# rlog58/dags-vae-search

Hardware: AMD Instinct MI355X
Metric: DAGs/sec VAE+predictor train step, n=12 batch 4096 per GPU, at 1 MI355X (higher is better)
Workload: dtype f32 (fwd bf16x6, bwd bf16x3 split products, fp32 accumulate); 1 GPU; synthetic_v12 DAGs (n=12, card=12, N=15 tokens), PACE-VAE train step: pack + fwd + bwd + clip_grad_norm_(1.0) + Adam(1e-4), train mode dropout 0.15; per_gpu_batch=4096, global_batch=4096, waves_per_workgroup=8, parallelism=single

## Files before the change

dags_vae_search_amd/csrc/dvs_api.hip:

```cpp
#include <math.h>
#include <stdarg.h>
#include <stdio.h>
#include <stdlib.h>
#include <string.h>

#include "dvs_kernels.h"
#include "dvs_backward.h"
#include "dvs_wide.h"
#include "dvs_wimg.h"
#include "dvs_decode.h"
#include "dvs_search_args.h"

static thread_local char g_err[256] = "";

#include <map>
#include <mutex>
#include <string>
#include <utility>
#include <vector>
namespace {
struct ProfRec {
    const char* name;
#ifndef DVS_EMU
    hipEvent_t a, b;
// ... 446 lines not shown
    return call_end("dvs_build_records");
}

static inline int slot_enc(int layer, int sub) { return 1 + 2 * layer + sub; }
static inline int slot_dec(int layer, int sub) { return 8 + 3 * layer + sub; }
static inline int site_enc(int layer, int k) { return 4 + 4 * layer + k; }
static inline int site_dec(int layer, int k) { return 16 + 6 * layer + k; }

static inline size_t img_attn(int block) { return (size_t)block * DvsAttnImg::SIZE; }
static inline size_t img_ffn(int block) { return DVS_N_ATTN_BLOCKS * DvsAttnImg::SIZE + (size_t)block * DvsFfnImg::SIZE; }
static inline int blk_enc_attn(int layer) { return layer; }
static inline int blk_dec_self(int layer) { return 3 + 2 * layer; }
static inline int blk_dec_cross(int layer) { return 4 + 2 * layer; }
static inline int blk_enc_ffn(int layer) { return layer; }
static inline int blk_dec_ffn(int layer) { return 3 + layer; }

static inline const void* wimg_attn(const Step& c, int block) { return (const dvs_bf16*)(c.ws + c.W.wimg) + img_attn(block); }
static inline const void* wimg_ffn(const Step& c, int block) { return (const dvs_bf16*)(c.ws + c.W.wimg) + img_ffn(block); }

static DvsLN ln_of(const Step& c, int slot, const DvsNormP* n) {
    if (!n) return DvsLN{nullptr, nullptr, nullptr};
    return DvsLN{c.ws + c.W.stats[slot], c.P + n->w, c.P + n->b};
}

static EmbedArgs embed_args(const Step& c, int site) {
    EmbedArgs e;
    memset(&e, 0, sizeof(e));
    e.dims = c.d;
    e.rec = c.rec;
    e.W1 = c.P + c.L.W1;
    e.W2 = c.P + c.L.W2;
    e.lab_w = c.P + c.L.lab_w;
    e.lab_b = c.P + c.L.lab_b;
    e.embimg = (const float*)((const dvs_bf16*)(c.ws + c.W.wimg) + DVS_WIMG_EMB);
    e.site = site;
    return e;
}

static AttnArgs attn_args(const Step& c, const DvsAttnP& p, int block, int in, const DvsNormP* norm, const float* kv, int out,
                          int site0) {
    AttnArgs a;
    memset(&a, 0, sizeof(a));
    a.dims = c.d;
    a.rec = c.rec;
    a.xin = c.ws + c.W.act[in];
    a.ln = ln_of(c, in, norm);
    a.kv = kv;
    a.in_w = c.P + p.in_w;
    a.in_b = c.P + p.in_b;
    a.out_w = c.P + p.out_w;
    a.out_b = c.P + p.out_b;
    a.wimg = wimg_attn(c, block);
    a.qkv = c.wide ? c.ws + c.W.qkv[block] : nullptr;
    a.out_pre = c.ws + c.W.act[out];
    a.out_stats = c.ws + c.W.stats[out];
    a.site_prob = site0;
    a.site_post = site0 + 1;
    return a;
}

static FfnArgs ffn_args(const Step& c, const DvsFfnP& p, int block, int in, const DvsNormP& norm, int out, int site0) {
    FfnArgs f;
    memset(&f, 0, sizeof(f));
    f.dims = c.d;
    f.xin = c.ws + c.W.act[in];
    f.ln = ln_of(c, in, &norm);
    f.l1_w = c.P + p.l1_w;
// ... 92 lines not shown
        attn(L.enc[i].sa, blk_enc_attn(i));
        ffn(L.enc[i].ff, blk_enc_ffn(i));
        attn(L.dec[i].sa, blk_dec_self(i));
        attn(L.dec[i].ca, blk_dec_cross(i));
        ffn(L.dec[i].ff, blk_dec_ffn(i));
    }
    if (!wide) {
        add(L.edge0_w, DVS_WIMG_LOSS + DvsLossImg::Wa, 64, 8);
        add(L.edge0_w + 64, DVS_WIMG_LOSS + DvsLossImg::Wb, 64, 8);
        add(L.edge0_w, DVS_WIMG_LOSS + DvsLossImg::WaT, 64, 8 | 1);
        add(L.edge0_w + 64, DVS_WIMG_LOSS + DvsLossImg::WbT, 64, 8 | 1);
    }
    dvs_bf16* wimg = (dvs_bf16*)(c.ws + c.W.wimg);
    DvsLatImgArgs lat;
    lat.fc1_w = c.P + L.fc1_w;
    lat.fc2_w = c.P + L.fc2_w;
    lat.fc3_w = c.P + L.fc3_w;
    lat.fc3_b = c.P + L.fc3_b;
    lat.img = c.ws + c.W.limg;
    lat.N = c.d.N;
    lat.NT = c.d.NT;
    DvsLossHeadArgs head;
    memset(&head, 0, sizeof(head));
    if (!wide) {
        head_params(c, head);
        head.ln_g = c.P + L.dec[DVS_LAYERS - 1].n3.w;
        head.ln_b = c.P + L.dec[DVS_LAYERS - 1].n3.b;
        head.dst = (float*)(wimg + DVS_WIMG_LOSS + DvsLossImg::Head);
        head.C = c.d.C;
        head.W1 = c.P + L.W1;
        head.W2 = c.P + L.W2;
        head.lab_w = c.P + L.lab_w;
        head.lab_b = c.P + L.lab_b;
        head.dst_emb = (float*)(wimg + DVS_WIMG_EMB);
        head.N = c.d.N;
    }
    dvs_launch_prepare_images(J, c.P, wimg, lat, head, c.st);
}

static void launch_embed_fwd(const Step& c, const EmbedArgs& e) {
    if (c.wide) dvs_launch_embed_fwd_w(e, c.g.tiles4, c.st);
    else if (c.nw == 4) dvs_launch_embed_fwd(e, c.g.chain, 4, c.st);
    else dvs_launch_embed_fwd(e, c.g.tiles16, 16, c.st);
}
static void launch_attn_fwd(const Step& c, const AttnArgs& a) {
    if (c.wide) dvs_launch_attn_fwd_w(a, c.g.dags, c.st);
    else if (c.nw == 4) dvs_launch_attn_fwd(a, c.g.chain, 4, c.st);
    else dvs_launch_attn_fwd(a, c.g.tiles8, 8, c.st);
}
static void launch_ffn_fwd(const Step& c, const FfnArgs& f) {
    if (c.nw == 4) dvs_launch_ffn_fwd(f, c.g.chain, 4, c.st);
    else dvs_launch_ffn_fwd(f, c.g.tiles16, 16, c.st);
}
static void launch_loss_fwd(const Step& c, const LossArgs& a) {
    if (c.wide) dvs_launch_loss_fwd_w(a, c.g.dags2, c.st);
    else if (c.nw == 4) dvs_launch_loss_fwd(a, c.g.chain, 4, c.st);
    else dvs_launch_loss_fwd(a, c.g.tiles8, 8, c.st);
}
struct FwdChain {
    FwdStackArgs stack;
    const Step& c;
    int tag;
    bool chain;
    FwdChain(const Step& step, int tag_) : c(step), tag(tag_), chain(!step.wide && !split_stack()) { memset(&stack, 0, sizeof(stack)); }
    FwdPhase& next(int kind) {
        if (stack.nphase == DVS_FWD_STACK_PHASES) flush();
        FwdPhase& ph = stack.ph[stack.nphase++];
// ... 221 lines not shown
```

dags_vae_search_amd/csrc/dvs_bf16.h:

```cpp
#pragma once
#include "dvs_device.h"

typedef __bf16 dvs_bf16;
typedef __bf16 bf8 __attribute__((ext_vector_type(8)));

constexpr int DVS_LDB = 72;

__device__ __forceinline__ f4 dvs_mfma_bf(bf8 a, bf8 b, f4 c) { return __builtin_amdgcn_mfma_f32_16x16x32_bf16(a, b, c, 0, 0, 0); }

__device__ __forceinline__ int dvs_kperm(int f) {
    const int t = f >> 4, g = (f >> 2) & 3, kk = f & 3;
    return 32 * (t >> 1) + 8 * g + 4 * (t & 1) + kk;
}

__device__ __forceinline__ void dvs_split1(float v, dvs_bf16& hi, dvs_bf16& lo) {
    hi = (dvs_bf16)v;
    lo = (dvs_bf16)(v - (float)hi);
}
__device__ __forceinline__ void dvs_split8(const f4& a, const f4& b, bf8& hi, bf8& lo) {
#pragma unroll
    for (int i = 0; i < 4; ++i) {
        dvs_bf16 h, l;
        dvs_split1(a[i], h, l);
        hi[i] = h;
        lo[i] = l;
        dvs_split1(b[i], h, l);
        hi[4 + i] = h;
        lo[4 + i] = l;
    }
}
struct SplitT {
    bf8 hi[2], lo[2];
};
__device__ __forceinline__ SplitT dvs_split_T(const f4 (&x)[4]) {
    SplitT s;
    dvs_split8(x[0], x[1], s.hi[0], s.lo[0]);
    dvs_split8(x[2], x[3], s.hi[1], s.lo[1]);
    return s;
}

__device__ __forceinline__ bf8 dvs_wfrag(const dvs_bf16* img, int row, int p, const Lane& L) {
    return *(const bf8*)(img + row * DVS_LDB + 32 * p + 8 * L.g);
}

template <int OT>
__device__ __forceinline__ void dvs_matb_T(f4 (&y)[OT], const SplitT& x, const dvs_bf16* Wh, const dvs_bf16* Wl, int row0,
                                           const Lane& L) {
#pragma unroll
    for (int p = 0; p < 2; ++p) {
        bf8 ah[OT], al[OT];
#pragma unroll
        for (int ot = 0; ot < OT; ++ot) {
            ah[ot] = dvs_wfrag(Wh, row0 + 16 * ot + L.r, p, L);
            al[ot] = dvs_wfrag(Wl, row0 + 16 * ot + L.r, p, L);
        }
#pragma unroll
        for (int ot = 0; ot < OT; ++ot) y[ot] = dvs_mfma_bf(ah[ot], x.hi[p], y[ot]);
#pragma unroll
        for (int ot = 0; ot < OT; ++ot) y[ot] = dvs_mfma_bf(ah[ot], x.lo[p], y[ot]);
#pragma unroll
        for (int ot = 0; ot < OT; ++ot) y[ot] = dvs_mfma_bf(al[ot], x.hi[p], y[ot]);
        DVS_SCHED_FENCE();
    }
}
template <int OT>
__device__ __forceinline__ void dvs_matb_N(f4 (&y)[OT], const SplitT& x, const dvs_bf16* Wh, const dvs_bf16* Wl, int row0,
                                           const Lane& L) {
#pragma unroll
    for (int p = 0; p < 2; ++p) {
        bf8 bh[OT], bl[OT];
#pragma unroll
        for (int ot = 0; ot < OT; ++ot) {
            bh[ot] = dvs_wfrag(Wh, row0 + 16 * ot + L.r, p, L);
            bl[ot] = dvs_wfrag(Wl, row0 + 16 * ot + L.r, p, L);
        }
#pragma unroll
        for (int ot = 0; ot < OT; ++ot) y[ot] = dvs_mfma_bf(x.hi[p], bh[ot], y[ot]);
#pragma unroll
        for (int ot = 0; ot < OT; ++ot) y[ot] = dvs_mfma_bf(x.lo[p], bh[ot], y[ot]);
#pragma unroll
        for (int ot = 0; ot < OT; ++ot) y[ot] = dvs_mfma_bf(x.hi[p], bl[ot], y[ot]);
        DVS_SCHED_FENCE();
    }
}

struct Split3T {
    bf8 hi[2], mid[2], lo[2];
// ... 18 lines not shown
            dvs_split3_1(x[2 * p + 1][i], h, m, l);
            s.hi[p][4 + i] = h;
            s.mid[p][4 + i] = m;
            s.lo[p][4 + i] = l;
        }
    return s;
}
template <int OT, bool N_LAYOUT = false>
__device__ __forceinline__ void dvs_matb3(f4 (&y)[OT], const Split3T& x, const dvs_bf16* img, int rows, int row0, const Lane& L) {
    const dvs_bf16* Wh = img;
    const dvs_bf16* Wm = img + rows * DVS_LDB;
    const dvs_bf16* Wl = Wm + rows * DVS_LDB;
#pragma unroll
    for (int p = 0; p < 2; ++p) {
        bf8 wh[OT], wm[OT], wl[OT];
#pragma unroll
        for (int ot = 0; ot < OT; ++ot) {
            wh[ot] = dvs_wfrag(Wh, row0 + 16 * ot + L.r, p, L);
            wm[ot] = dvs_wfrag(Wm, row0 + 16 * ot + L.r, p, L);
            wl[ot] = dvs_wfrag(Wl, row0 + 16 * ot + L.r, p, L);
        }
#define DVS_M3(wa, xa)                                                                                     \
    _Pragma("unroll") for (int ot = 0; ot < OT; ++ot)                                                      \
        y[ot] = N_LAYOUT ? dvs_mfma_bf(xa[p], wa[ot], y[ot]) : dvs_mfma_bf(wa[ot], xa[p], y[ot]);
        DVS_M3(wl, x.hi)
        DVS_M3(wh, x.lo)
        DVS_M3(wm, x.mid)
        DVS_M3(wm, x.hi)
        DVS_M3(wh, x.mid)
        DVS_M3(wh, x.hi)
#undef DVS_M3
        DVS_SCHED_FENCE();
    }
}

typedef __bf16 bf4 __attribute__((ext_vector_type(4)));
constexpr int DVS_PLD = 68;
constexpr int DVS_PKB = 16 * DVS_PLD;

__device__ __forceinline__ void dvs_park_bf(dvs_bf16* img, const f4 (&x)[4], const Lane& L) {
#pragma unroll
    for (int t = 0; t < 4; ++t) {
        bf4 h, l;
#pragma unroll
        for (int i = 0; i < 4; ++i) {
            dvs_bf16 hh, ll;
            dvs_split1(x[t][i], hh, ll);
            h[i] = hh;
            l[i] = ll;
        }
        *(bf4*)(img + L.r * DVS_PLD + 16 * t + 4 * L.g) = h;
        *(bf4*)(img + DVS_PKB + L.r * DVS_PLD + 16 * t + 4 * L.g) = l;
    }
}
__device__ __forceinline__ bf4 dvs_tr_read(const dvs_bf16* p) {
#ifndef DVS_EMU
    typedef short s4_ __attribute__((ext_vector_type(4)));
    const s4_ v = __builtin_amdgcn_ds_read_tr16_b64_v4i16((s4_ __attribute__((address_space(3)))*)p);
    return __builtin_bit_cast(bf4, v);
#else
    const unsigned long long a = (unsigned long long)p;
    const int lane = (int)(threadIdx.x & 63), grp = lane & 48, i = lane & 15;
    bf4 out;
    for (int q = 0; q < 4; ++q) {
        const int src = grp + 4 * q + (i >> 2);
        const unsigned lo = __shfl((unsigned)(a & 0xFFFFFFFFull), src), hi = __shfl((unsigned)(a >> 32), src);
// ... 47 lines not shown
```

dags_vae_search_amd/csrc/dvs_kernels.h:

```cpp
#pragma once
#include "dvs_device.h"
#include "dvs_host.h"
#include "dvs_stage.h"

#ifndef DVS_EMU
typedef hipStream_t dvs_stream_t;
#else
typedef void* dvs_stream_t;
#endif

struct DvsLN {
    const float* stats;
    const float* g;
    const float* b;
};

struct PackArgs {
    int B, N, C;
    const float* lab1h;
    const float* pos1h;
    const float* adj;
    const uint8_t* tmask;
    DvsRecord* rec;
    int* status;
};

struct EmbedArgs {
    DvsDims dims;
    const DvsRecord* rec;
    const float *W1, *W2, *lab_w, *lab_b;
    const float* embimg;
    float* out;
    int site;
    float* out2;
    int site2;
    const float* gout;
    float* slab;
    int64_t P;
    int64_t oW1, oW2, olab_w, olab_b;
};

struct AttnArgs {
    DvsDims dims;
    const DvsRecord* rec;
    const float* xin;
    DvsLN ln;
    const float* kv;
    const float *in_w, *in_b, *out_w, *out_b;
    const void* wimg;
    float* out_pre;
    float* out_stats;
    int site_prob, site_post;
    float* qkv;
};

struct FfnArgs {
    DvsDims dims;
    const float* xin;
    DvsLN ln;
    const float *l1_w, *l1_b, *l2_w, *l2_b;
    const void* wimg;
    float* out_pre;
    float* out_stats;
    float* out_norm;
// ... 236 lines not shown
```

dags_vae_search_amd/csrc/dvs_wimg.h:

```cpp
#pragma once
#include "dvs_bf16.h"

constexpr size_t DVS_IMG64 = 64 * (size_t)DVS_LDB;
struct DvsAttnImg {
    static constexpr size_t Win = 0;
    static constexpr size_t Wout = 3 * 3 * DVS_IMG64;
    static constexpr size_t WoutT = Wout + 3 * DVS_IMG64;
    static constexpr size_t WinB = WoutT + 2 * DVS_IMG64;
    static constexpr size_t WinT = WinB + 2 * 3 * DVS_IMG64;
    static constexpr size_t SIZE = WinT + 3 * 2 * DVS_IMG64;
};
struct DvsFfnImg {
    static constexpr size_t W2T = 0;
    static constexpr size_t W1T = 2 * DVS_IMG64;
    static constexpr size_t W1 = 4 * DVS_IMG64;
    static constexpr size_t W2 = 7 * DVS_IMG64;
    static constexpr size_t SIZE = 10 * DVS_IMG64;
};
struct DvsLossImg {
    static constexpr size_t Wa = 0;
    static constexpr size_t Wb = 3 * DVS_IMG64;
    static constexpr size_t WaT = 6 * DVS_IMG64;
    static constexpr size_t WbT = 8 * DVS_IMG64;
    static constexpr size_t Head = 10 * DVS_IMG64;
    static constexpr int HEAD_FLOATS = 32 * 68 + 16 * 36 + 32 + 16 + 64 + 64 + 16 + 64 + 64;
    static constexpr size_t SIZE = Head + 2 * (size_t)HEAD_FLOATS;
};
static_assert(DvsLossImg::HEAD_FLOATS % 256 == 0 && DVS_LD == 68, "whole 1 KB chunks (dvs_stage.h)");
struct DvsEmbImg {
    static constexpr int FLOATS = 5120;
};
struct DvsLossHeadArgs {
    const float *node0_w, *node0_b, *node2_w, *node2_b, *edge0_b, *edge2_w, *edge2_b, *ln_g, *ln_b;
    float* dst;
    int C;
    const float *W1, *W2, *lab_w, *lab_b;
    float* dst_emb;
    int N;
};
constexpr int DVS_N_ATTN_BLOCKS = 9, DVS_N_FFN_BLOCKS = 6;
constexpr size_t DVS_WIMG_LOSS = DVS_N_ATTN_BLOCKS * DvsAttnImg::SIZE + DVS_N_FFN_BLOCKS * DvsFfnImg::SIZE;
constexpr size_t DVS_WIMG_EMB = DVS_WIMG_LOSS + DvsLossImg::SIZE;
constexpr size_t DVS_WIMG_BF16 = DVS_WIMG_EMB + 2 * (size_t)DvsEmbImg::FLOATS;

struct DvsLatImg {
    static constexpr size_t LD(int NT) { return (size_t)1024 * NT + 64; }
    static constexpr size_t A(int) { return 0; }
    static constexpr size_t AT(int NT) { return 64 * LD(NT); }
    static constexpr size_t W3(int NT) { return AT(NT) + (size_t)64 * 1024 * NT; }
    static constexpr size_t W3T(int NT) { return W3(NT) + (size_t)32 * 1024 * NT; }
    static constexpr size_t B3(int NT) { return W3T(NT) + 32 * LD(NT); }
    static constexpr size_t floats(int NT) { return B3(NT) + (size_t)1024 * NT; }
};
struct DvsLatImgArgs {
    const float *fc1_w, *fc2_w, *fc3_w, *fc3_b;
    float* img;
    int N, NT;
};

struct DvsImgJob {
    int64_t src;
    int64_t dst;
    int32_t rows;
    int32_t flags;
};
constexpr int DVS_MAX_IMG_JOBS = 96;
struct DvsImgJobs {
    DvsImgJob job[DVS_MAX_IMG_JOBS];
    int count;
};
void dvs_launch_prepare_images(const DvsImgJobs& jobs, const float* params, dvs_bf16* wimg, const DvsLatImgArgs& lat,
                               const DvsLossHeadArgs& head, dvs_stream_t st);

__device__ __forceinline__ void dvs_copy_image(dvs_bf16* dst, const dvs_bf16* __restrict__ src, int n) {
    const f4* s = (const f4*)src;
    f4* d = (f4*)dst;
// ... 31 lines not shown
```

dags_vae_search_amd/csrc/k_backward_heads.hip:

```cpp
#include "dvs_backward.h"
#include "dvs_wimg.h"
#include "dvs_latent_bwd.h"
#include "dvs_loss.h"

#ifdef DVS_STAMPS
__device__ unsigned long long dvs_stamps_lossb[256 * 4 * 12];
DVS_STAMP_READER(lossb)
#endif
#define LBSTAMP(k) DVS_ACC_STAMP_AT(dvs_stamps_lossb, lst_, 4, 12, k)
template <bool EMIT>
__global__ __launch_bounds__(256) void k_loss_bwd(LossArgs a, DvsStagePlan plan) {
#ifdef DVS_STAMPS
    unsigned long long lst_ = __builtin_amdgcn_s_memtime();
#endif
    DVS_DYN_LDS(smem);
    const LossLds l = loss_lds(smem);
    const int N = a.dims.N, C = a.dims.C;
    dvs_stage_now<(LOSS_CHUNKS + 3) / 4>(&plan, smem);
    __syncthreads();
    const Lane L = dvs_lane();
    float* scrV = l.scr + L.wave * 3 * DVS_SCR;
    float* scrU = scrV + DVS_SCR;
    float* dlm = scrU + DVS_SCR;
    const float b2 = l.b2[0];
// ... 228 lines not shown
        const float sb2 = dvs_sum_wave(L.g == 0 ? db2 : 0.f);
        float* rb2 = rv + 192 + 4 * DVS_RED_VEC;
        if (L.lane == 0) rb2[L.wave] = sb2;
        __syncthreads();
        dvs_flush_dw<2, 4>(rN1, slab + a.o_node0_w, L);
        dvs_flush_dw<1, 2>(rN2, slab + a.o_node2_w, L, C, 32);
        dvs_flush_vec<2>(rv, slab + a.o_node0_b, L);
        dvs_flush_vec<1>(rv + 128, slab + a.o_node2_b, L, C);
        dvs_flush_vec<4>(rv + 192 + DVS_RED_VEC, slab + a.o_edge2_w, L);
        dvs_flush_vec<4>(rv + 192 + 2 * DVS_RED_VEC, slab + a.o_ln_g, L);
        dvs_flush_vec<4>(rv + 192 + 3 * DVS_RED_VEC, slab + a.o_ln_b, L);
        if (threadIdx.x == 0) {
            float s = rb2[0];
            for (int w = 1; w < L.nwaves; ++w) s += rb2[w];
            slab[a.o_edge2_b] = s;
        }
    }
    LBSTAMP(9);
}

void dvs_launch_loss_bwd(const LossArgs& a, int grid, bool emit_loss, dvs_stream_t st) {
    const size_t lds = loss_lds_bytes(4, 3);
    DvsStagePlan plan;
    loss_plan(plan, a);
    if (emit_loss) {
        DVS_SET_LDS(k_loss_bwd<true>, lds);
        DVS_LAUNCH_AS("k_loss_bwd", k_loss_bwd<true>, dim3(grid), dim3(256), lds, st, a, plan);
    } else {
        DVS_SET_LDS(k_loss_bwd<false>, lds);
        DVS_LAUNCH_AS("k_loss_bwd", k_loss_bwd<false>, dim3(grid), dim3(256), lds, st, a, plan);
    }
}

__global__ __launch_bounds__(512) void k_embed_bwd(EmbedArgs a, const float* gout2, int site2, DvsStagePlan plan) {
    DVS_DYN_LDS(smem);
    const int N = a.dims.N, C = a.dims.C;
    float* W1 = (float*)smem;
    float* W2 = W1 + 2 * DVS_MAXTOK * DVS_LD;
    float* labw = W2 + 64 * EMB_LDW2;
    float* labb = labw + 32 * 16;
    float* scr0 = labb + 32;
    if (blockDim.x >= 512) dvs_stage_now<3>(&plan, smem);
    else dvs_stage_now<5>(&plan, smem);
    __syncthreads();
    const Lane L = dvs_lane();
    const DvsDrop D = dvs_drop_of(a.dims);
    float* scr = scr0 + L.wave * DVS_SCR;
    f4 dW2[4][2], dlabb[2], dW1a[1][4], dW1b[1][4], dlab[2][1];
#pragma unroll
    for (int i = 0; i < 4; ++i) dW2[i][0] = dW2[i][1] = dW1a[0][i] = dW1b[0][i] = f4_zero();
    dlabb[0] = dlabb[1] = dlab[0][0] = dlab[1][0] = f4_zero();
    for (int dag = blockIdx.x * L.nwaves + L.wave; dag < a.dims.B; dag += gridDim.x * L.nwaves) {
        const DvsRecord* rec = a.rec + dag;
        const bool valid = L.r < N;
        const int label = rec->label[L.r];
        const uint32_t gdag = a.dims.dag_offset + dag;
        const EmbSel sel = dvs_emb_selectors(rec, N, scr, L);
        f4 e1[4];
        dvs_emb_hidden(e1, W1, N, sel, L);
        for (int src = 0; src < 2; ++src) {
            const float* gsrc = src == 0 ? a.gout : gout2;
            if (!gsrc) continue;
            const int site = src == 0 ? a.site : site2;
            f4 gx[4];
            dvs_load_grad(gx, gsrc, dag, N, L);
            f4 dle[2];
#pragma unroll
            for (int t = 0; t < 2; ++t)
#pragma unroll
                for (int kk = 0; kk < 4; ++kk) {
                    const int f = 16 * t + 4 * L.g + kk;
                    const float pre = labw[f * 16 + label] + labb[f];
                    dle[t][kk] = (valid && pre > 0.f) ? gx[t][kk] : 0.f;
                }
            dlabb[0] += dle[0];
            dlabb[1] += dle[1];
            const uint32_t k1 = dvs_site_key(a.dims.seed_lo, a.dims.seed_hi, site, gdag);
            f4 m1[4] = {f4_splat(1.f), f4_splat(1.f), f4_splat(1.f), f4_splat(1.f)};
            dvs_dropout_tile(m1, k1, D, L);
            f4 e1d[4];
#pragma unroll
            for (int t = 0; t < 4; ++t) e1d[t] = e1[t] * m1[t];
            f4 de2[2] = {gx[2], gx[3]};
            dvs_dropout_tile<2>(de2, dvs_site_key(a.dims.seed_lo, a.dims.seed_hi, site + 1, gdag), D, L);
            f4 e1dN[4], de2N[2], dleN[2];
            dvs_t2n<4>(e1dN, e1d, scr, L);
            dvs_t2n<2>(de2N, de2, scr, L);
            dvs_t2n<2>(dleN, dle, scr, L);
            dvs_outer_acc<4, 2>(dW2, e1dN, de2N);
            f4 de1[4] = {f4_zero(), f4_zero(), f4_zero(), f4_zero()};
            dvs_mat_T<4, 2>(de1, de2, W2, EMB_LDW2, 0, L);
#pragma unroll
            for (int t = 0; t < 4; ++t) de1[t] *= m1[t];
#pragma unroll
            for (int t = 0; t < 4; ++t)
#pragma unroll
                for (int kk = 0; kk < 4; ++kk) de1[t][kk] = e1[t][kk] > 0.f ? de1[t][kk] : 0.f;
            f4 de1N[4];
            dvs_t2n<4>(de1N, de1, scr, L);
            f4 selA[1] = {sel.selA}, parA[1] = {sel.parA}, labA[1] = {sel.labA};
            dvs_outer_acc<1, 4>(dW1a, selA, de1N);
            dvs_outer_acc<1, 4>(dW1b, parA, de1N);
            dvs_outer_acc<2, 1>(dlab, dleN, labA);
        }
    }
    __syncthreads();
    float* slab = a.slab + (size_t)blockIdx.x * a.P;
    float* r1a = (float*)smem;
    float* r1b = r1a + 8 * 1024;
    float* rlab = r1b + 8 * 1024;
    float* rv = rlab + 8 * 512;
    dvs_stage_dw<1, 4>(r1a, dW1a, L);
    dvs_stage_dw<1, 4>(r1b, dW1b, L);
    dvs_stage_dw<2, 1>(rlab, dlab, L);
    dvs_stage_vec<2>(rv, dlabb, rv + 8 * 32 + L.wave * DVS_SCR, L);
    __syncthreads();
    dvs_flush_dw<1, 4>(r1a, slab + a.oW1, L, N, 64);
    dvs_flush_dw<1, 4>(r1b, slab + a.oW1 + (size_t)N * 64, L, N, 64);
    dvs_flush_dw<2, 1>(rlab, slab + a.olab_w, L, 32, C, C);
    dvs_flush_vec<2>(rv, slab + a.olab_b, L);
    __syncthreads();
    float* rW2 = (float*)smem;
    dvs_stage_dw<4, 2>(rW2, dW2, L);
    __syncthreads();
    dvs_flush_dw<4, 2>(rW2, slab + a.oW2, L);
}

void dvs_launch_embed_bwd(const EmbedArgs& a, const float* gout2, int site2, int grid, int nw, dvs_stream_t st) {
    size_t lds = (2 * DVS_MAXTOK * DVS_LD + 64 * EMB_LDW2 + 32 * 16 + 32 + 8 * DVS_SCR) * 4;
    const size_t red = (8 * (1024 + 1024 + 512) + 8 * 32 + 8 * DVS_SCR) * 4;
    if (lds < red) lds = red;
    DvsStagePlan plan;
    dvs_plan_clear(plan);
    dvs_plan_seg(plan, DVS_FAKE_LDS, DVS_FAKE_LDS, a.embimg, 2 * DvsEmbImg::FLOATS);
    dvs_plan_seal(plan);
    DVS_SET_LDS(k_embed_bwd, lds);
    DVS_LAUNCH(k_embed_bwd, dim3(grid), dim3(nw == 4 ? 256 : 512), lds, st, a, gout2, site2, plan);
}

constexpr int LATB_WAVES = 8;
__global__ __launch_bounds__(64 * LATB_WAVES) void k_latent_bwd(LatentBwdArgs a) {
    __shared__ f4 part[LATB_WAVES][2][64];
    dvs_latent_bwd_group<LATB_WAVES>(a, part, (int)blockIdx.x * 16, (int)blockIdx.x * 16 + 8);
}

void dvs_launch_latent_bwd(const LatentBwdArgs& a, dvs_stream_t st) {
    const int ngroups = (a.dims.B + 15) / 16;
    DVS_LAUNCH(k_latent_bwd, dim3(ngroups), dim3(64 * LATB_WAVES), 0, st, a);
}

constexpr int FC_MT = 4;
__global__ __launch_bounds__(512) void k_fc_dw(FcDwArgs a) {
    __shared__ f4 red[4][FC_MT * 6 + 2][64];
    const Lane L = dvs_lane();
    const int B = a.dims.B, N = a.dims.N;
    const int ldw = N * 64;
    const int nmg = 16 * a.dims.NT;
    const int mg = blockIdx.x % nmg, q = blockIdx.x / nmg;
    const size_t dstride = (size_t)a.dims.NT * DVS_TILE;
    const int per_q = (B + DVS_FC_PARTS - 1) / DVS_FC_PARTS;
    const int per_w = (per_q + 7) / 8;
    const int d0 = q * per_q + L.wave * per_w;
    int d1 = d0 + per_w;
    if (d1 > (q + 1) * per_q) d1 = (q + 1) * per_q;
    if (d1 > B) d1 = B;
    f4 acc[FC_MT][4], acc3[FC_MT][2];
    f4 bs3 = f4_zero();
// ... 130 lines not shown
```

dags_vae_search_amd/csrc/k_forward.hip:

```cpp
#include "dvs_kernels.h"
#include "dvs_wimg.h"

constexpr int PACK_DAGS = 4;
__device__ __forceinline__ void pack_stream(float* dst, const float* __restrict__ src, size_t nfloats) {
    const size_t n4 = nfloats >> 2;
    size_t i = threadIdx.x;
    for (; i + 3 * blockDim.x < n4; i += 4 * blockDim.x) {
        f4 v[4];
#pragma unroll
        for (int u = 0; u < 4; ++u) v[u] = *(const f4*)(src + 4 * (i + u * blockDim.x));
#pragma unroll
        for (int u = 0; u < 4; ++u) *(f4*)(dst + 4 * (i + u * blockDim.x)) = v[u];
    }
    for (; i < n4; i += blockDim.x) *(f4*)(dst + 4 * i) = *(const f4*)(src + 4 * i);
    for (size_t i = 4 * n4 + threadIdx.x; i < nfloats; i += blockDim.x) dst[i] = src[i];
}
__global__ __launch_bounds__(8 * 16 * PACK_DAGS) void k_pack(PackArgs a) {
    DVS_DYN_LDS(smem);
    const int N = a.N, C = a.C;
    const int dag0 = blockIdx.x * PACK_DAGS;
    const int nd = (a.B - dag0 < PACK_DAGS) ? a.B - dag0 : PACK_DAGS;
    float* s_lab = (float*)smem;
    float* s_pos = s_lab + PACK_DAGS * 16 * 16;
    float* s_adj = s_pos + PACK_DAGS * 16 * 16;
// ... 139 lines not shown
        unsigned parents = 0, allowed = 1u << i;
        if (i < N) {
            if (i == 0) label = 2;
            else if (i == 1) label = 0;
            else if (i == out_id) label = 1;
            else {
                label = a.labels[(size_t)dag * n + (i - 2)] + 3;
                if (label >= a.C) { bad |= 1; label = 0; }
            }
            pos = s_order[i][tid];
            allowed = 0;
            for (int j = 0; j < N; ++j) {
                if ((s_child[j][tid] >> i) & 1u) parents |= 1u << j;
                if ((s_reach[j][tid] >> i) & 1u) allowed |= 1u << j;
            }
        }
        r->label[i] = (uint8_t)label;
        r->pos[i] = (uint8_t)pos;
        r->parents[i] = (uint16_t)parents;
        r->allowed[i] = (uint16_t)allowed;
    }
    if (bad) atomicOr(a.status, bad);
}

void dvs_launch_build_records(const BuildArgs& a, dvs_stream_t st) {
    DVS_LAUNCH(k_build_records, dim3((a.B + 255) / 256), dim3(256), 0, st, a);
}

struct EmbLds {
    float *W1, *W2, *labw, *labb, *scr;
};
__device__ __forceinline__ EmbLds emb_lds(char* smem) {
    EmbLds l;
    l.W1 = (float*)smem;
    l.W2 = l.W1 + 2 * DVS_MAXTOK * DVS_LD;
    l.labw = l.W2 + 64 * EMB_LDW2;
    l.labb = l.labw + 32 * 16;
    l.scr = l.labb + 32;
    return l;
}
static size_t emb_lds_floats(int nwaves) {
    const size_t n = 2 * DVS_MAXTOK * DVS_LD + 64 * EMB_LDW2 + 32 * 16 + 32 + (size_t)nwaves * 16;
    return n > (size_t)DvsEmbImg::FLOATS ? n : (size_t)DvsEmbImg::FLOATS;
}

__global__ __launch_bounds__(1024) void k_embed_fwd(EmbedArgs a, DvsStagePlan plan) {
    DVS_DYN_LDS(smem);
    const int N = a.dims.N, C = a.dims.C;
    const EmbLds l = emb_lds(smem);
    if (blockDim.x >= 1024) dvs_stage_now<2>(&plan, smem);
    else dvs_stage_now<5>(&plan, smem);
    __syncthreads();
    const Lane L = dvs_lane();
    const DvsDrop D = dvs_drop_of(a.dims);
    float* scr = l.scr + L.wave * 16;
    for (int dag = blockIdx.x * L.nwaves + L.wave; dag < a.dims.B; dag += gridDim.x * L.nwaves) {
        const DvsRecord* rec = a.rec + dag;
        const bool valid = L.r < N;
        const EmbSel sel = dvs_emb_selectors(rec, N, scr, L);
        f4 eh[4];
        dvs_emb_hidden(eh, l.W1, N, sel, L);
        const uint32_t gdag = a.dims.dag_offset + dag;
        const int label = rec->label[L.r];
        for (int v = 0; v < (a.out2 ? 2 : 1); ++v) {
            const int site = v ? a.site2 : a.site;
            f4 e1[4];
#pragma unroll
            for (int t = 0; t < 4; ++t) e1[t] = eh[t];
            dvs_dropout_tile(e1, dvs_site_key(a.dims.seed_lo, a.dims.seed_hi, site, gdag), D, L);
            f4 x[4];
            f4 e2[2] = {f4_zero(), f4_zero()};
#pragma unroll
            for (int t = 0; t < 4; ++t) {
                const f4 w0 = dvs_wcol(l.W2, EMB_LDW2, 0, t, L), w1 = dvs_wcol(l.W2, EMB_LDW2, 16, t, L);
#pragma unroll
                for (int kk = 0; kk < 4; ++kk) {
                    e2[0] = dvs_mfma(w0[kk], e1[t][kk], e2[0]);
                    e2[1] = dvs_mfma(w1[kk], e1[t][kk], e2[1]);
                }
            }
            {
                f4 tmp[2] = {e2[0], e2[1]};
                dvs_dropout_tile<2>(tmp, dvs_site_key(a.dims.seed_lo, a.dims.seed_hi, site + 1, gdag), D, L);
                x[2] = tmp[0];
                x[3] = tmp[1];
            }
#pragma unroll
            for (int t = 0; t < 2; ++t)
#pragma unroll
                for (int kk = 0; kk < 4; ++kk) {
                    const int f = 16 * t + 4 * L.g + kk;
                    x[t][kk] = valid ? fmaxf(l.labw[f * 16 + label] + l.labb[f], 0.f) : 0.f;
                }
            if (!valid) { x[2] = f4_zero(); x[3] = f4_zero(); }
            dvs_store_tile(v ? a.out2 : a.out, dag, x, L);
        }
    }
}

void dvs_launch_embed_fwd(const EmbedArgs& a, int grid, int nw, dvs_stream_t st) {
    const size_t lds = emb_lds_floats(16) * 4;
    DvsStagePlan plan;
    dvs_plan_clear(plan);
    dvs_plan_seg(plan, DVS_FAKE_LDS, DVS_FAKE_LDS, a.embimg, 2 * DvsEmbImg::FLOATS);
    dvs_plan_seal(plan);
    DVS_SET_LDS(k_embed_fwd, lds);
    DVS_LAUNCH(k_embed_fwd, dim3(grid), dim3(nw == 4 ? 256 : 1024), lds, st, a, plan);
}

#ifdef DVS_STAMPS
DVS_STAMP_DECL(dvs_stamps_fwd);
struct DvsLatTag { int phase; };
__device__ const DvsLatTag dvs_lat_tag = {6};
#define DVS_LAT_STAMP(id) DVS_STAMP(dvs_stamps_fwd, &dvs_lat_tag, id)
DVS_ACC_STAMP_DECL(dvs_stamps_attn);
#endif
#define ASTAMP(k) DVS_ACC_STAMP(dvs_stamps_attn, ast_, k)
#include "dvs_latent.h"
struct AttnLds {
    dvs_bf16 *Win, *Wout;
    float *inb, *outb, *lg, *lb;
};
DVS_HD inline AttnLds attn_lds(char* smem) {
    AttnLds l;
    l.Win = (dvs_bf16*)smem;
    l.Wout = l.Win + 3 * 192 * DVS_LDB;
    l.inb = (float*)(l.Wout + 3 * 64 * DVS_LDB);
    l.outb = l.inb + 192;
    l.lg = l.outb + 64;
    l.lb = l.lg + 64;
    return l;
}
static size_t attn_lds_bytes() { return 3 * 256 * DVS_LDB * sizeof(dvs_bf16) + (192 + 64 + 128) * sizeof(float); }

inline void attn_plan(DvsStagePlan& p, const AttnArgs& a, char* smem) {
    const AttnLds l = attn_lds(smem);
    dvs_plan_clear(p);
// ... 396 lines not shown
```

dags_vae_search_amd/csrc/k_optim.hip:

```cpp
#include "dvs_backward.h"

constexpr int SQ_PARTS = 256;
__global__ __launch_bounds__(256) void k_sqnorm_part(const float* g, int64_t n, float* scratch) {
    __shared__ float part[256];
    float s = 0.f;
    const int64_t n4 = n >> 2;
    for (int64_t i = (int64_t)blockIdx.x * 256 + threadIdx.x; i < n4; i += (int64_t)SQ_PARTS * 256) {
        const f4 v = *(const f4*)(g + 4 * i);
        s += (v[0] * v[0] + v[1] * v[1]) + (v[2] * v[2] + v[3] * v[3]);
    }
    if (blockIdx.x == 0)
        for (int64_t i = 4 * n4 + threadIdx.x; i < n; i += 256) s += g[i] * g[i];
    part[threadIdx.x] = s;
    __syncthreads();
    for (int k = 128; k > 0; k >>= 1) {
        if ((int)threadIdx.x < k) part[threadIdx.x] += part[threadIdx.x + k];
        __syncthreads();
    }
    if (threadIdx.x == 0) scratch[2 + blockIdx.x] = part[0];
}
__global__ __launch_bounds__(256) void k_adam(int64_t n, float* p, float* g, float* m, float* v, float lr, float b1, float b2,
                                              float eps, float bc1, float bc2_sqrt, float max_norm, float* scratch,
                                              const float* guard, int nparts) {
    __shared__ float part[256];
// ... 35 lines not shown
                          dvs_stream_t st) {
    if (!have_partials) DVS_LAUNCH(k_sqnorm_part, dim3(SQ_PARTS), dim3(256), 0, st, (const float*)grads, n, scratch);
    const float bc1 = 1.0f - powf(b1, (float)step);
    const float bc2 = 1.0f - powf(b2, (float)step);
    DVS_LAUNCH(k_adam, dim3((unsigned)((n + 255) / 256)), dim3(256), 0, st, n, params, grads, m, v, lr, b1, b2, eps,
                       bc1, sqrtf(bc2), max_norm, scratch, guard, have_partials ? dvs_sq_parts(n) : SQ_PARTS);
}

#include "dvs_wimg.h"
__device__ __forceinline__ float dvs_loss_head_value(const DvsLossHeadArgs& h, int i) {
    if (i < 32 * 68) {
        const int r = i / 68, c = i % 68;
        return c < 64 ? h.node0_w[r * 64 + c] : 0.f;
    }
    i -= 32 * 68;
    if (i < 16 * 36) {
        const int c = i / 36, k = i % 36;
        return (c < h.C && k < 32) ? h.node2_w[c * 32 + k] : 0.f;
    }
    i -= 16 * 36;
    if (i < 32) return h.node0_b[i];
    i -= 32;
    if (i < 16) return i < h.C ? h.node2_b[i] : 0.f;
    i -= 16;
    if (i < 64) return h.edge0_b[i];
    i -= 64;
    if (i < 64) return h.edge2_w[i];
    i -= 64;
    if (i < 16) return i == 0 ? h.edge2_b[0] : 0.f;
    i -= 16;
    if (i < 64) return h.ln_g[i];
    return h.ln_b[i - 64];
}
__device__ __forceinline__ float dvs_emb_block_value(const DvsLossHeadArgs& h, int i) {
    if (i < 32 * 68) {
        const int r = i / 68, c = i % 68;
        return (r < 2 * h.N && c < 64) ? h.W1[r * 64 + c] : 0.f;
    }
    i -= 32 * 68;
    if (i < 64 * 36) {
        const int f = i / 36, k = i % 36;
        return k < 32 ? h.W2[f * 32 + k] : 0.f;
    }
    i -= 64 * 36;
    if (i < 512) {
        const int f = i >> 4, c = i & 15;
        return c < h.C ? h.lab_w[f * h.C + c] : 0.f;
    }
    i -= 512;
    return i < 32 ? h.lab_b[i] : 0.f;
}
__global__ __launch_bounds__(256) void k_prepare_images(DvsImgJobs jobs, const float* params, dvs_bf16* wimg, DvsLatImgArgs lat,
                                                        DvsLossHeadArgs head) {
    const int nlat = 1024 * lat.NT / 64;
    const int first_job = nlat + (head.dst ? 2 : 0);
    if (head.dst) {
        if ((int)blockIdx.x == nlat + 1) {
            float v[DvsEmbImg::FLOATS / 256];
#pragma unroll
            for (int u = 0; u < DvsEmbImg::FLOATS / 256; ++u) v[u] = dvs_emb_block_value(head, u * 256 + (int)threadIdx.x);
#pragma unroll
            for (int u = 0; u < DvsEmbImg::FLOATS / 256; ++u) head.dst_emb[u * 256 + threadIdx.x] = v[u];
            return;
        }
        if ((int)blockIdx.x == nlat) {
            float v[DvsLossImg::HEAD_FLOATS / 256];
#pragma unroll
            for (int u = 0; u < DvsLossImg::HEAD_FLOATS / 256; ++u) v[u] = dvs_loss_head_value(head, u * 256 + (int)threadIdx.x);
#pragma unroll
            for (int u = 0; u < DvsLossImg::HEAD_FLOATS / 256; ++u) head.dst[u * 256 + threadIdx.x] = v[u];
            return;
        }
    }
    if ((int)blockIdx.x < nlat) {
        __shared__ float tile[64][65];
        const int K = 1024 * lat.NT, kp0 = (int)blockIdx.x * 64;
        const int l = threadIdx.x & 63, w = threadIdx.x >> 6;
        const size_t ldw = (size_t)lat.N * 64;
        auto col_of = [&](int kp, bool& valid) {
            const int tile_i = kp >> 10, q = (kp & 1023) >> 2, kk = kp & 3, t = q >> 6, ln = q & 63;
            const int tok = 16 * tile_i + (ln & 15), feat = 16 * t + 4 * (ln >> 4) + kk;
            valid = tok < lat.N;
            return (size_t)(valid ? tok : 0) * 64 + feat;
        };
        bool valid;
        const size_t col = col_of(kp0 + l, valid);
        float va[16];
#pragma unroll
        for (int i = 0; i < 16; ++i) {
            const int o = w + 4 * i;
            va[i] = !valid ? 0.f : (o < 32 ? lat.fc1_w[o * ldw + col] : lat.fc2_w[(o - 32) * ldw + col]);
        }
        float v3[8];
#pragma unroll
        for (int i = 0; i < 8; ++i) {
// ... 19 lines not shown
        }
        __syncthreads();
        for (int o = w; o < 32; o += 4) lat.img[DvsLatImg::W3T(lat.NT) + (size_t)o * DvsLatImg::LD(lat.NT) + kp0 + l] = tile[o][l];
        if (w == 0) lat.img[DvsLatImg::B3(lat.NT) + kp0 + l] = vb3;
        return;
    }
    const int jb = ((int)blockIdx.x - first_job) / 12, slice = ((int)blockIdx.x - first_job) % 12;
    const DvsImgJob J = jobs.job[jb];
    const bool transposed = J.flags & 1, rperm = J.flags & 2, cperm = J.flags & 4;
    const float* src = params + J.src;
    dvs_bf16* dst = wimg + J.dst;
    for (int i = threadIdx.x; i < 16 * 64; i += blockDim.x) {
        const int row = 16 * slice + (i >> 6), col = i & 63;
        if (row >= J.rows) break;
        const float v = src[(size_t)(rperm ? dvs_pi(row) : row) * ((J.flags & 8) ? 128 : 64) + (cperm ? dvs_pi(col) : col)];
        if (!transposed) {
            dvs_bf16 h, m, l;
            dvs_split3_1(v, h, m, l);
            const size_t o = (size_t)row * DVS_LDB + dvs_kperm(col), part = (size_t)J.rows * DVS_LDB;
            dst[o] = h;
            dst[part + o] = m;
            if (!(J.flags & 16)) dst[2 * part + o] = l;
        } else {
            dvs_bf16 h, l;
            dvs_split1(v, h, l);
            const size_t o = (size_t)col * DVS_LDB + dvs_kperm(row);
            dst[o] = h;
            dst[DVS_IMG64 + o] = l;
        }
    }
}
void dvs_launch_prepare_images(const DvsImgJobs& jobs, const float* params, dvs_bf16* wimg, const DvsLatImgArgs& lat,
                               const DvsLossHeadArgs& head, dvs_stream_t st) {
    DVS_LAUNCH(k_prepare_images, dim3(jobs.count * 12 + 1024 * lat.NT / 64 + (head.dst ? 2 : 0)), dim3(256), 0, st, jobs, params,
               wimg, lat, head);
}
```

Baseline: 3.467 million DAGs/s.

## Use bf16 split MFMA for embed backward and add transposed W2 bf16 image

The embedding backward kernel's weight-gradient outer products and the de1 = W2^T·de2 product now use bf16 hi/lo split MFMA (bf16x3) instead of the fp32 path. To support this, the embedding weight image is re-laid out: the fp32 W2 block comes first, followed by W1 and the label weights, then a new bf16 hi/lo transposed W2 block. The forward and backward kernels each stage only the segment they need. The image-preparation kernel builds this mixed layout across 16 workgroups instead of one. This trades fp32 FMA throughput for matrix-core throughput, at some precision risk, and makes the image layout more complex.

```diff
diff --git a/dags_vae_search_amd/csrc/dvs_api.hip b/dags_vae_search_amd/csrc/dvs_api.hip
--- a/dags_vae_search_amd/csrc/dvs_api.hip
+++ b/dags_vae_search_amd/csrc/dvs_api.hip
@@ -502,7 +502,7 @@
     e.W2 = c.P + c.L.W2;
     e.lab_w = c.P + c.L.lab_w;
     e.lab_b = c.P + c.L.lab_b;
-    e.embimg = (const float*)((const dvs_bf16*)(c.ws + c.W.wimg) + DVS_WIMG_EMB);
+    e.embimg = (const dvs_bf16*)(c.ws + c.W.wimg) + DVS_WIMG_EMB;
     e.site = site;
     return e;
 }
@@ -661,7 +661,7 @@
         head.W2 = c.P + L.W2;
         head.lab_w = c.P + L.lab_w;
         head.lab_b = c.P + L.lab_b;
-        head.dst_emb = (float*)(wimg + DVS_WIMG_EMB);
+        head.dst_emb = wimg + DVS_WIMG_EMB;
         head.N = c.d.N;
     }
     dvs_launch_prepare_images(J, c.P, wimg, lat, head, c.st);
diff --git a/dags_vae_search_amd/csrc/dvs_bf16.h b/dags_vae_search_amd/csrc/dvs_bf16.h
--- a/dags_vae_search_amd/csrc/dvs_bf16.h
+++ b/dags_vae_search_amd/csrc/dvs_bf16.h
@@ -39,20 +39,20 @@
     return s;
 }
 
-__device__ __forceinline__ bf8 dvs_wfrag(const dvs_bf16* img, int row, int p, const Lane& L) {
-    return *(const bf8*)(img + row * DVS_LDB + 32 * p + 8 * L.g);
-}
-
-template <int OT>
+__device__ __forceinline__ bf8 dvs_wfrag(const dvs_bf16* img, int row, int p, const Lane& L, int ld = DVS_LDB) {
+    return *(const bf8*)(img + row * ld + 32 * p + 8 * L.g);
+}
+
+template <int OT, int KB = 2>
 __device__ __forceinline__ void dvs_matb_T(f4 (&y)[OT], const SplitT& x, const dvs_bf16* Wh, const dvs_bf16* Wl, int row0,
-                                           const Lane& L) {
-#pragma unroll
-    for (int p = 0; p < 2; ++p) {
+                                           const Lane& L, int ld = DVS_LDB) {
+#pragma unroll
+    for (int p = 0; p < KB; ++p) {
         bf8 ah[OT], al[OT];
 #pragma unroll
         for (int ot = 0; ot < OT; ++ot) {
-            ah[ot] = dvs_wfrag(Wh, row0 + 16 * ot + L.r, p, L);
-            al[ot] = dvs_wfrag(Wl, row0 + 16 * ot + L.r, p, L);
+            ah[ot] = dvs_wfrag(Wh, row0 + 16 * ot + L.r, p, L, ld);
+            al[ot] = dvs_wfrag(Wl, row0 + 16 * ot + L.r, p, L, ld);
         }
 #pragma unroll
         for (int ot = 0; ot < OT; ++ot) y[ot] = dvs_mfma_bf(ah[ot], x.hi[p], y[ot]);
@@ -137,6 +137,69 @@
 #undef DVS_M3
         DVS_SCHED_FENCE();
     }
+}
+
+struct SplitN {
+    bf8 hi, lo;
+};
+__device__ __forceinline__ bf8 dvs_exact_N(const f4& v) {
+    bf8 e;
+#pragma unroll
+    for (int i = 0; i < 4; ++i) {
+        e[i] = (dvs_bf16)v[i];
+        e[4 + i] = (dvs_bf16)0.0f;
+    }
+    return e;
+}
+__device__ __forceinline__ SplitN dvs_split_N(const f4& v) {
+    SplitN s;
+#pragma unroll
+    for (int i = 0; i < 4; ++i) {
+        dvs_bf16 h, l;
+        dvs_split1(v[i], h, l);
+        s.hi[i] = h;
+        s.lo[i] = l;
+        s.hi[4 + i] = (dvs_bf16)0.0f;
+        s.lo[4 + i] = (dvs_bf16)0.0f;
+    }
+    return s;
+}
+template <int OT, int IT>
+__device__ __forceinline__ void dvs_outer_acc_bf(f4 (&dw)[OT][IT], const SplitN (&a)[OT], const SplitN (&b)[IT]) {
+#pragma unroll
+    for (int ot = 0; ot < OT; ++ot)
+#pragma unroll
+        for (int it = 0; it < IT; ++it) dw[ot][it] = dvs_mfma_bf(a[ot].lo, b[it].hi, dw[ot][it]);
+#pragma unroll
+    for (int ot = 0; ot < OT; ++ot)
+#pragma unroll
+        for (int it = 0; it < IT; ++it) dw[ot][it] = dvs_mfma_bf(a[ot].hi, b[it].lo, dw[ot][it]);
+#pragma unroll
+    for (int ot = 0; ot < OT; ++ot)
+#pragma unroll
+        for (int it = 0; it < IT; ++it) dw[ot][it] = dvs_mfma_bf(a[ot].hi, b[it].hi, dw[ot][it]);
+}
+template <int OT, int IT>
+__device__ __forceinline__ void dvs_outer_acc_bf(f4 (&dw)[OT][IT], const bf8 (&a)[OT], const SplitN (&b)[IT]) {
+#pragma unroll
+    for (int ot = 0; ot < OT; ++ot)
+#pragma unroll
+        for (int it = 0; it < IT; ++it) dw[ot][it] = dvs_mfma_bf(a[ot], b[it].lo, dw[ot][it]);
+#pragma unroll
+    for (int ot = 0; ot < OT; ++ot)
+#pragma unroll
+        for (int it = 0; it < IT; ++it) dw[ot][it] = dvs_mfma_bf(a[ot], b[it].hi, dw[ot][it]);
+}
+template <int OT, int IT>
+__device__ __forceinline__ void dvs_outer_acc_bf(f4 (&dw)[OT][IT], const SplitN (&a)[OT], const bf8 (&b)[IT]) {
+#pragma unroll
+    for (int ot = 0; ot < OT; ++ot)
+#pragma unroll
+        for (int it = 0; it < IT; ++it) dw[ot][it] = dvs_mfma_bf(a[ot].lo, b[it], dw[ot][it]);
+#pragma unroll
+    for (int ot = 0; ot < OT; ++ot)
+#pragma unroll
+        for (int it = 0; it < IT; ++it) dw[ot][it] = dvs_mfma_bf(a[ot].hi, b[it], dw[ot][it]);
 }
 
 typedef __bf16 bf4 __attribute__((ext_vector_type(4)));
diff --git a/dags_vae_search_amd/csrc/dvs_kernels.h b/dags_vae_search_amd/csrc/dvs_kernels.h
--- a/dags_vae_search_amd/csrc/dvs_kernels.h
+++ b/dags_vae_search_amd/csrc/dvs_kernels.h
@@ -29,7 +29,7 @@
     DvsDims dims;
     const DvsRecord* rec;
     const float *W1, *W2, *lab_w, *lab_b;
-    const float* embimg;
+    const void* embimg;
     float* out;
     int site;
     float* out2;
diff --git a/dags_vae_search_amd/csrc/dvs_wimg.h b/dags_vae_search_amd/csrc/dvs_wimg.h
--- a/dags_vae_search_amd/csrc/dvs_wimg.h
+++ b/dags_vae_search_amd/csrc/dvs_wimg.h
@@ -28,20 +28,30 @@
 };
 static_assert(DvsLossImg::HEAD_FLOATS % 256 == 0 && DVS_LD == 68, "whole 1 KB chunks (dvs_stage.h)");
 struct DvsEmbImg {
-    static constexpr int FLOATS = 5120;
+    static constexpr int LDH = 40;
+    static constexpr size_t W2 = 0;
+    static constexpr size_t W1 = 2 * 64 * 36;
+    static constexpr size_t Lab = W1 + 2 * 32 * 68;
+    static constexpr size_t W2T = Lab + 2 * (32 * 16 + 32);
+    static constexpr size_t END = W2T + 2 * 64 * LDH;
+    static constexpr size_t FWD_N = (W2T + 511) / 512 * 512;
+    static constexpr size_t BWD_N = (END - W1 + 511) / 512 * 512;
+    static constexpr size_t SIZE = W1 + BWD_N;
 };
+static_assert(DvsEmbImg::W1 % 8 == 0 && DvsEmbImg::Lab % 8 == 0 && DvsEmbImg::W2T % 8 == 0 && DvsEmbImg::FWD_N <= DvsEmbImg::SIZE &&
+              DVS_LD == 68, "16-byte aligned parts; the forward's segment ends inside the block");
 struct DvsLossHeadArgs {
     const float *node0_w, *node0_b, *node2_w, *node2_b, *edge0_b, *edge2_w, *edge2_b, *ln_g, *ln_b;
     float* dst;
     int C;
     const float *W1, *W2, *lab_w, *lab_b;
-    float* dst_emb;
+    dvs_bf16* dst_emb;
     int N;
 };
 constexpr int DVS_N_ATTN_BLOCKS = 9, DVS_N_FFN_BLOCKS = 6;
 constexpr size_t DVS_WIMG_LOSS = DVS_N_ATTN_BLOCKS * DvsAttnImg::SIZE + DVS_N_FFN_BLOCKS * DvsFfnImg::SIZE;
 constexpr size_t DVS_WIMG_EMB = DVS_WIMG_LOSS + DvsLossImg::SIZE;
-constexpr size_t DVS_WIMG_BF16 = DVS_WIMG_EMB + 2 * (size_t)DvsEmbImg::FLOATS;
+constexpr size_t DVS_WIMG_BF16 = DVS_WIMG_EMB + DvsEmbImg::SIZE;
 
 struct DvsLatImg {
     static constexpr size_t LD(int NT) { return (size_t)1024 * NT + 64; }
diff --git a/dags_vae_search_amd/csrc/k_backward_heads.hip b/dags_vae_search_amd/csrc/k_backward_heads.hip
--- a/dags_vae_search_amd/csrc/k_backward_heads.hip
+++ b/dags_vae_search_amd/csrc/k_backward_heads.hip
@@ -284,16 +284,17 @@
     }
 }
 
+constexpr int EMB_BWD_CHUNKS = (int)(DvsEmbImg::BWD_N / 512);
 __global__ __launch_bounds__(512) void k_embed_bwd(EmbedArgs a, const float* gout2, int site2, DvsStagePlan plan) {
     DVS_DYN_LDS(smem);
     const int N = a.dims.N, C = a.dims.C;
-    float* W1 = (float*)smem;
-    float* W2 = W1 + 2 * DVS_MAXTOK * DVS_LD;
-    float* labw = W2 + 64 * EMB_LDW2;
-    float* labb = labw + 32 * 16;
-    float* scr0 = labb + 32;
-    if (blockDim.x >= 512) dvs_stage_now<3>(&plan, smem);
-    else dvs_stage_now<5>(&plan, smem);
+    const float* W1 = (const float*)smem;
+    const float* labw = W1 + 2 * DVS_MAXTOK * DVS_LD;
+    const float* labb = labw + 32 * 16;
+    const dvs_bf16* W2T = (const dvs_bf16*)smem + (DvsEmbImg::W2T - DvsEmbImg::W1);
+    float* scr0 = (float*)(smem + 2 * DvsEmbImg::BWD_N);
+    if (blockDim.x >= 512) dvs_stage_now<(EMB_BWD_CHUNKS + 7) / 8>(&plan, smem);
+    else dvs_stage_now<(EMB_BWD_CHUNKS + 3) / 4>(&plan, smem);
     __syncthreads();
     const Lane L = dvs_lane();
     const DvsDrop D = dvs_drop_of(a.dims);
@@ -339,9 +340,19 @@
             dvs_t2n<4>(e1dN, e1d, scr, L);
             dvs_t2n<2>(de2N, de2, scr, L);
             dvs_t2n<2>(dleN, dle, scr, L);
-            dvs_outer_acc<4, 2>(dW2, e1dN, de2N);
+            SplitN de2S[2] = {dvs_split_N(de2N[0]), dvs_split_N(de2N[1])};
+            {
+                SplitN e1dS[4];
+#pragma unroll
+                for (int t = 0; t < 4; ++t) e1dS[t] = dvs_split_N(e1dN[t]);
+                dvs_outer_acc_bf<4, 2>(dW2, e1dS, de2S);
+            }
             f4 de1[4] = {f4_zero(), f4_zero(), f4_zero(), f4_zero()};
-            dvs_mat_T<4, 2>(de1, de2, W2, EMB_LDW2, 0, L);
+            {
+                SplitT de2T;
+                dvs_split8(de2[0], de2[1], de2T.hi[0], de2T.lo[0]);
+                dvs_matb_T<4, 1>(de1, de2T, W2T, W2T + 64 * DvsEmbImg::LDH, 0, L, DvsEmbImg::LDH);
+            }
 #pragma unroll
             for (int t = 0; t < 4; ++t) de1[t] *= m1[t];
 #pragma unroll
@@ -350,10 +361,14 @@
                 for (int kk = 0; kk < 4; ++kk) de1[t][kk] = e1[t][kk] > 0.f ? de1[t][kk] : 0.f;
             f4 de1N[4];
             dvs_t2n<4>(de1N, de1, scr, L);
-            f4 selA[1] = {sel.selA}, parA[1] = {sel.parA}, labA[1] = {sel.labA};
-            dvs_outer_acc<1, 4>(dW1a, selA, de1N);
-            dvs_outer_acc<1, 4>(dW1b, parA, de1N);
-            dvs_outer_acc<2, 1>(dlab, dleN, labA);
+            const bf8 selA[1] = {dvs_exact_N(sel.selA)}, parA[1] = {dvs_exact_N(sel.parA)}, labA[1] = {dvs_exact_N(sel.labA)};
+            SplitN de1S[4];
+#pragma unroll
+            for (int t = 0; t < 4; ++t) de1S[t] = dvs_split_N(de1N[t]);
+            dvs_outer_acc_bf<1, 4>(dW1a, selA, de1S);
+            dvs_outer_acc_bf<1, 4>(dW1b, parA, de1S);
+            const SplitN dleS[2] = {dvs_split_N(dleN[0]), dvs_split_N(dleN[1])};
+            dvs_outer_acc_bf<2, 1>(dlab, dleS, labA);
         }
     }
     __syncthreads();
@@ -379,12 +394,12 @@
 }
 
 void dvs_launch_embed_bwd(const EmbedArgs& a, const float* gout2, int site2, int grid, int nw, dvs_stream_t st) {
-    size_t lds = (2 * DVS_MAXTOK * DVS_LD + 64 * EMB_LDW2 + 32 * 16 + 32 + 8 * DVS_SCR) * 4;
+    size_t lds = DvsEmbImg::BWD_N * 2 + 8 * DVS_SCR * 4;
     const size_t red = (8 * (1024 + 1024 + 512) + 8 * 32 + 8 * DVS_SCR) * 4;
     if (lds < red) lds = red;
     DvsStagePlan plan;
     dvs_plan_clear(plan);
-    dvs_plan_seg(plan, DVS_FAKE_LDS, DVS_FAKE_LDS, a.embimg, 2 * DvsEmbImg::FLOATS);
+    dvs_plan_seg(plan, DVS_FAKE_LDS, DVS_FAKE_LDS, (const dvs_bf16*)a.embimg + DvsEmbImg::W1, (int)DvsEmbImg::BWD_N);
     dvs_plan_seal(plan);
     DVS_SET_LDS(k_embed_bwd, lds);
     DVS_LAUNCH(k_embed_bwd, dim3(grid), dim3(nw == 4 ? 256 : 512), lds, st, a, gout2, site2, plan);
diff --git a/dags_vae_search_amd/csrc/k_forward.hip b/dags_vae_search_amd/csrc/k_forward.hip
--- a/dags_vae_search_amd/csrc/k_forward.hip
+++ b/dags_vae_search_amd/csrc/k_forward.hip
@@ -195,17 +195,18 @@
 };
 __device__ __forceinline__ EmbLds emb_lds(char* smem) {
     EmbLds l;
-    l.W1 = (float*)smem;
-    l.W2 = l.W1 + 2 * DVS_MAXTOK * DVS_LD;
-    l.labw = l.W2 + 64 * EMB_LDW2;
+    l.W2 = (float*)smem;
+    l.W1 = l.W2 + 64 * EMB_LDW2;
+    l.labw = l.W1 + 2 * DVS_MAXTOK * DVS_LD;
     l.labb = l.labw + 32 * 16;
     l.scr = l.labb + 32;
     return l;
 }
 static size_t emb_lds_floats(int nwaves) {
     const size_t n = 2 * DVS_MAXTOK * DVS_LD + 64 * EMB_LDW2 + 32 * 16 + 32 + (size_t)nwaves * 16;
-    return n > (size_t)DvsEmbImg::FLOATS ? n : (size_t)DvsEmbImg::FLOATS;
-}
+    return n > DvsEmbImg::FWD_N / 2 ? n : DvsEmbImg::FWD_N / 2;
+}
+static_assert(DvsEmbImg::FWD_N == 20 * 512, "k_embed_fwd stages 20 wave chunks");
 
 __global__ __launch_bounds__(1024) void k_embed_fwd(EmbedArgs a, DvsStagePlan plan) {
     DVS_DYN_LDS(smem);
@@ -265,7 +266,7 @@
     const size_t lds = emb_lds_floats(16) * 4;
     DvsStagePlan plan;
     dvs_plan_clear(plan);
-    dvs_plan_seg(plan, DVS_FAKE_LDS, DVS_FAKE_LDS, a.embimg, 2 * DvsEmbImg::FLOATS);
+    dvs_plan_seg(plan, DVS_FAKE_LDS, DVS_FAKE_LDS, (const dvs_bf16*)a.embimg + DvsEmbImg::W2, (int)DvsEmbImg::FWD_N);
     dvs_plan_seal(plan);
     DVS_SET_LDS(k_embed_fwd, lds);
     DVS_LAUNCH(k_embed_fwd, dim3(grid), dim3(nw == 4 ? 256 : 1024), lds, st, a, plan);
diff --git a/dags_vae_search_amd/csrc/k_optim.hip b/dags_vae_search_amd/csrc/k_optim.hip
--- a/dags_vae_search_amd/csrc/k_optim.hip
+++ b/dags_vae_search_amd/csrc/k_optim.hip
@@ -91,35 +91,74 @@
     if (i < 64) return h.ln_g[i];
     return h.ln_b[i - 64];
 }
-__device__ __forceinline__ float dvs_emb_block_value(const DvsLossHeadArgs& h, int i) {
-    if (i < 32 * 68) {
-        const int r = i / 68, c = i % 68;
-        return (r < 2 * h.N && c < 64) ? h.W1[r * 64 + c] : 0.f;
-    }
-    i -= 32 * 68;
-    if (i < 64 * 36) {
-        const int f = i / 36, k = i % 36;
-        return k < 32 ? h.W2[f * 32 + k] : 0.f;
-    }
-    i -= 64 * 36;
-    if (i < 512) {
-        const int f = i >> 4, c = i & 15;
-        return c < h.C ? h.lab_w[f * h.C + c] : 0.f;
-    }
-    i -= 512;
-    return i < 32 ? h.lab_b[i] : 0.f;
-}
+__device__ __forceinline__ int dvs_kperm_inv(int c) {
+    const int t = 2 * (c >> 5) + ((c >> 2) & 1), g = (c >> 3) & 3, kk = c & 3;
+    return 16 * t + 4 * g + kk;
+}
+struct DvsEmbSrc {
+    const float* p;
+    bool live;
+    int part;
+};
+__device__ __forceinline__ DvsEmbSrc dvs_emb_src(const DvsLossHeadArgs& h, int e) {
+    constexpr int LDH = DvsEmbImg::LDH;
+    DvsEmbSrc s;
+    s.part = -1;
+    if (e < (int)DvsEmbImg::W1) {
+        const int i = e >> 1, f = i / 36, k = i % 36;
+        s.live = k < 32;
+        s.p = h.W2 + f * 32 + (k < 32 ? k : 0);
+    } else if (e < (int)DvsEmbImg::Lab) {
+        const int i = (e - (int)DvsEmbImg::W1) >> 1, r = i / 68, c = i % 68;
+        s.live = r < 2 * h.N && c < 64;
+        s.p = h.W1 + (s.live ? r * 64 + c : 0);
+    } else if (e < (int)DvsEmbImg::W2T) {
+        const int i = (e - (int)DvsEmbImg::Lab) >> 1, f = (i >> 4) & 31, c = i & 15;
+        s.live = i >= 512 || c < h.C;
+        s.p = i < 512 ? h.lab_w + f * h.C + (c < h.C ? c : 0) : h.lab_b + (i - 512);
+    } else {
+        const int i = e - (int)DvsEmbImg::W2T;
+        const bool in = i < 2 * 64 * LDH;
+        s.part = in ? i / (64 * LDH) : 0;
+        const int f = (i % (64 * LDH)) / LDH, c = i % LDH;
+        s.live = in && c < 32;
+        s.p = h.W2 + f * 32 + dvs_kperm_inv(c < 32 ? c : 0);
+    }
+    return s;
+}
+__device__ __forceinline__ unsigned short dvs_emb_part(const DvsEmbSrc& s, float v) {
+    dvs_bf16 hi, lo;
+    dvs_split1(v, hi, lo);
+    return __builtin_bit_cast(unsigned short, s.part <= 0 ? hi : lo);
+}
+constexpr int DVS_EMB_WORDS = (int)(DvsEmbImg::SIZE / 2);
+constexpr int DVS_EMB_WGS = 16;
+constexpr int DVS_EMB_WPT = (DVS_EMB_WORDS + DVS_EMB_WGS * 256 - 1) / (DVS_EMB_WGS * 256);
 __global__ __launch_bounds__(256) void k_prepare_images(DvsImgJobs jobs, const float* params, dvs_bf16* wimg, DvsLatImgArgs lat,
                                                         DvsLossHeadArgs head) {
     const int nlat = 1024 * lat.NT / 64;
-    const int first_job = nlat + (head.dst ? 2 : 0);
+    const int first_job = nlat + (head.dst ? 1 + DVS_EMB_WGS : 0);
     if (head.dst) {
-        if ((int)blockIdx.x == nlat + 1) {
-            float v[DvsEmbImg::FLOATS / 256];
-#pragma unroll
-            for (int u = 0; u < DvsEmbImg::FLOATS / 256; ++u) v[u] = dvs_emb_block_value(head, u * 256 + (int)threadIdx.x);
-#pragma unroll
-            for (int u = 0; u < DvsEmbImg::FLOATS / 256; ++u) head.dst_emb[u * 256 + threadIdx.x] = v[u];
+        if ((int)blockIdx.x > nlat && (int)blockIdx.x < first_job) {
+            const int w0 = (((int)blockIdx.x - nlat - 1) * DVS_EMB_WPT) * 256 + (int)threadIdx.x;
+            DvsEmbSrc s[DVS_EMB_WPT][2];
+            float v[DVS_EMB_WPT][2];
+#pragma unroll
+            for (int u = 0; u < DVS_EMB_WPT; ++u) {
+                const int w = w0 + u * 256, wc = w < DVS_EMB_WORDS ? w : DVS_EMB_WORDS - 1;
+#pragma unroll
+                for (int q = 0; q < 2; ++q) {
+                    s[u][q] = dvs_emb_src(head, 2 * wc + q);
+                    v[u][q] = *s[u][q].p;
+                }
+            }
+#pragma unroll
+            for (int u = 0; u < DVS_EMB_WPT; ++u) {
+                const float v0 = s[u][0].live ? v[u][0] : 0.f, v1 = s[u][1].live ? v[u][1] : 0.f;
+                const uint32_t word = s[u][0].part < 0 ? __builtin_bit_cast(uint32_t, v0)
+                                                       : (uint32_t)dvs_emb_part(s[u][0], v0) | ((uint32_t)dvs_emb_part(s[u][1], v1) << 16);
+                if (w0 + u * 256 < DVS_EMB_WORDS) ((uint32_t*)head.dst_emb)[w0 + u * 256] = word;
+            }
             return;
         }
         if ((int)blockIdx.x == nlat) {
@@ -205,6 +244,6 @@
 }
 void dvs_launch_prepare_images(const DvsImgJobs& jobs, const float* params, dvs_bf16* wimg, const DvsLatImgArgs& lat,
                                const DvsLossHeadArgs& head, dvs_stream_t st) {
-    DVS_LAUNCH(k_prepare_images, dim3(jobs.count * 12 + 1024 * lat.NT / 64 + (head.dst ? 2 : 0)), dim3(256), 0, st, jobs, params,
+    DVS_LAUNCH(k_prepare_images, dim3(jobs.count * 12 + 1024 * lat.NT / 64 + (head.dst ? 1 + DVS_EMB_WGS : 0)), dim3(256), 0, st, jobs, params,
                wimg, lat, head);
 }
```

Result: no change. 3.482 million DAGs/s, median of 6 (+0.4%).
